# zellerlab/GECCO

Measured on AMD Instinct MI355X. Metric: genes/sec CRF decode (windowed fwd-bwd marginals + Viterbi), higher is better.
Workload: dtype f64

## Files before the change

gecco_amd/build.py:

```python
import os
import shutil
import subprocess
import sys

HERE = os.path.dirname(os.path.abspath(__file__))
CSRC = os.path.join(HERE, "csrc")
LIBDIR = os.path.join(HERE, "lib")
LIB = os.path.join(LIBDIR, "libgecco_crf.so")
SOURCES = ["crf_model.cpp", "crf_plan.cpp", "crf_session.cpp", "crf_tables.cpp", "capi.cpp", "crf_kernels.hip", "crf_sequence.hip", "crf_segment.hip", "crf_general.hip", "crf_general_windowed.hip", "crf_spans.hip", "crf_conditionals.hip", "crf_runs.hip", "crf_sample.hip", "crf_kbest.hip", "crf_minrun.hip", "crf_counts.hip", "crf_edges.hip", "crf_composition.hip", "crf_exact.hip", "crf_train.hip", "crf_train_general.hip", "crf_fisher.hip", "crf_overlap.hip", "crf_forest.hip"]
HEADERS = ["crf_model.hpp", "crf_plan.hpp", "crf_device.hpp", "crf_scan.hpp", "crf_lanes.hpp", "crf_lane_group.hpp", "crf_contig_walk.hpp", "crf_vd_short.hpp", "crf_session.hpp", "crf_tables.hpp", "crf_exact_exp.hpp", "crf_npsum.hpp", "crf_train.hpp", "crf_train_host.hpp", "crf_hip_own.hpp", "crf_fisher.hpp", "crf_overlap.hpp", "crf_forest.hpp", os.path.join("..", "..", "include", "gecco_crf.h")]
EXTRA_FLAGS = {"crf_exact.hip": ["-ffp-contract=off"], "capi.cpp": ["-ffp-contract=off"], "crf_fisher.hip": ["-ffp-contract=off"],
               "crf_forest.hip": ["-ffp-contract=off"],
               "crf_spans.hip": ["-ffp-contract=off"],
               "crf_runs.hip": ["-ffp-contract=off"],
               "crf_conditionals.hip": ["-ffp-contract=off"],
               "crf_sample.hip": ["-ffp-contract=off"],
               "crf_kbest.hip": ["-ffp-contract=off"], "crf_minrun.hip": ["-ffp-contract=off"], "crf_counts.hip": ["-ffp-contract=off"]}
ARCH = "gfx950"


def _hipcc() -> str:
    for cand in (os.environ.get("HIPCC"), shutil.which("hipcc"), "/opt/rocm/bin/hipcc"):
        if cand and os.path.exists(cand):
            return cand
    raise RuntimeError("hipcc not found (ROCm toolchain required to build gecco_amd)")


def needs_build() -> bool:
    if not os.path.exists(LIB):
        return True
    t = os.path.getmtime(LIB)
    deps = [os.path.join(CSRC, s) for s in SOURCES + HEADERS] + [os.path.abspath(__file__)]
    return any(os.path.getmtime(d) > t for d in deps)


LAST_BUILD = {}


def build_native(force: bool = False, verbose: bool = False) -> str:
    if not force and not needs_build():
        LAST_BUILD["libgecco_crf"] = "reused (up to date against every source and header)"
        return LIB
    os.makedirs(LIBDIR, exist_ok=True)
# ... 58 lines not shown
```

gecco_amd/csrc/crf_vd_short.hpp:

```cpp
#pragma once

#include "crf_device.hpp"
#include "crf_scan.hpp"

namespace gecco {
namespace {

constexpr int kT = 256;
constexpr int kGPL = kSeqGenesPerLane;
constexpr int kBlockGenes = kT * kGPL;
static_assert(kBlockGenes == kSeqBlockGenes, "host tables assume this block size");

__device__ __forceinline__ double vd_max(double a, double b) {
    double r;
    asm("v_max_f64 %0, %1, %2" : "=v"(r) : "v"(a), "v"(b));
    return r;
}
__device__ __forceinline__ double vd_min(double a, double b) {
    double r;
    asm("v_min_f64 %0, %1, %2" : "=v"(r) : "v"(a), "v"(b));
    return r;
}
__device__ __forceinline__ double vd_min_abs(double a, double b) {
    double r;
    asm("v_min_f64 %0, |%1|, |%2|" : "=v"(r) : "v"(a), "v"(b));
    return r;
}
__device__ __forceinline__ double vd_max_s(double a, double bound) {
    double r;
    asm("v_max_f64 %0, %1, %2" : "=v"(r) : "v"(a), "s"(bound));
    return r;
}
__device__ __forceinline__ double vd_min_s(double a, double bound) {
    double r;
    asm("v_min_f64 %0, %1, %2" : "=v"(r) : "v"(a), "s"(bound));
    return r;
}
__device__ __forceinline__ void vd_shift_in_gt(uint32_t &acc, double x, double bound) {
    asm("v_cmp_lt_f64 vcc, %2, %1\n\tv_addc_co_u32 %0, vcc, %0, %0, vcc" : "+v"(acc) : "v"(x), "s"(bound) : "vcc");
}
struct COp {
    static __device__ __forceinline__ CE identity() { return CE{0.0, -__builtin_huge_val(), __builtin_huge_val()}; }
    static __device__ __forceinline__ CE combine(const CE &a, const CE &b) {
        return CE{a.a + b.a, vd_min(vd_max(a.L + b.a, b.L), b.H), vd_min(vd_max(a.H + b.a, b.L), b.H)};
    }
    static __device__ __forceinline__ void combine_into(CE &t, CE &v) {
        asm volatile(
            "v_add_f64 %[tl], %[tl], %[a]\n\t"
            "v_add_f64 %[th], %[th], %[a]\n\t"
            "v_add_f64 %[a], %[ta], %[a]\n\t"
            "v_max_f64 %[tl], %[tl], %[L]\n\t"
            "v_max_f64 %[th], %[th], %[L]\n\t"
            "v_min_f64 %[L], %[tl], %[H]\n\t"
            "v_min_f64 %[H], %[th], %[H]"
            : [a] "+v"(v.a), [L] "+v"(v.L), [H] "+v"(v.H), [tl] "+v"(t.L), [th] "+v"(t.H)
            : [ta] "v"(t.a));
    }
};

__device__ __forceinline__ double vd_bound(const SeqArgs &A, double nnz, double n) { return nnz * A.v_wmax2 + (n + 2.0) * A.v_tmax; }
constexpr double kVdEps = 2.220446049250313e-16;
__device__ __forceinline__ double vd_margin(double r, double ulpM) { return (4.0 * r + 4.0) * ulpM; }
__device__ __forceinline__ double vd_sum_slack(const SeqArgs &A, double nnz) {
    return (nnz * nnz + 3.0 * nnz + 1.0) * A.v_wmax2 * (0.5 * kVdEps) * 1.000001;
}

constexpr int kFixChunk = 1024;
struct FixStage {
    double2 st[kFixChunk];
    uint32_t bpw[kFixChunk / 16];
};
__device__ __forceinline__ void exact_states(const SeqArgs &A, int g0, int m, FixStage &fx, int first_lane) {
// ... 119 lines not shown
__device__ __forceinline__ void exact_delta_contig(const SeqArgs &A, int gs, int ge, FixStage &fx) {
    uint32_t *bpc = exact_bp_words(A, gs);
    double d0 = 0.0, d1 = 0.0;
    for (int cb = gs; cb < ge; cb += kFixChunk) {
        const int m = min(kFixChunk, ge - cb);
        const double e0 = d0, e1 = d1;
        exact_states(A, cb, m, fx, 0);
        __syncthreads();
        if (threadIdx.x == 0) exact_walk(A, fx, m, cb == gs, d0, d1);
        __syncthreads();
        d0 = fx.st[m - 1].x;
        d1 = fx.st[m - 1].y;
        exact_backpointers(A, fx, m, cb == gs, e0, e1);
        __syncthreads();
        for (int i = threadIdx.x; i < (m + 15) / 16; i += kT) bpc[(cb - gs) / 16 + i] = fx.bpw[i];
        __syncthreads();
    }
    exact_backtrack(A, gs, ge, d0, d1);
}

constexpr double kVdPad = 1e30;

struct VdShortSmem {
    double st[kT * (kGPL + 1)];
    uint32_t mark[kBlockGenes / 32];
    int c_end;
    CE tot[kT / 64];
    uint32_t mtot[kT / 64];
    double pv[kT / 64];
    uint32_t pbad[kT / 64];
    uint32_t vote[kT / 64];
};
static_assert(sizeof(VdShortSmem) <= 20480, "eight workgroups per CU");
__device__ __forceinline__ void load_short(const double *__restrict__ v, int g0, int n, VdShortSmem &stg, double (&x)[kGPL]) {
    const int base = int(threadIdx.x) * kGPL;
    const double *vp = v + g0;
    double *row = stg.st + threadIdx.x * (kGPL + 1);
    const int wave_end = (__builtin_amdgcn_readfirstlane(int(threadIdx.x >> 6)) + 1) * 64 * kGPL;
    if (wave_end <= n) {
#pragma unroll
        for (int k = 0; k < kGPL; ++k) x[k] = vp[base + k];
#pragma unroll
        for (int k = 0; k < kGPL; ++k) row[k] = x[k];
        return;
    }
#pragma unroll
    for (int k = 0; k < kGPL; ++k) x[k] = vp[max(min(base + k, n - 1), 0)];
#pragma unroll
    for (int k = 0; k < kGPL; ++k) {
        x[k] = base + k < n ? x[k] : kVdPad;
        row[k] = x[k];
    }
}

__device__ __forceinline__ uint32_t wave_or_u32(uint32_t v) {
    v |= uint32_t(__builtin_amdgcn_update_dpp(0, int(v), 0x111, 0xF, 0xF, true));
    v |= uint32_t(__builtin_amdgcn_update_dpp(0, int(v), 0x112, 0xF, 0xF, true));
    v |= uint32_t(__builtin_amdgcn_update_dpp(0, int(v), 0x114, 0xF, 0xF, true));
    v |= uint32_t(__builtin_amdgcn_update_dpp(0, int(v), 0x118, 0xF, 0xF, true));
    v |= uint32_t(__builtin_amdgcn_update_dpp(0, int(v), 0x142, 0xA, 0xF, true));
    v |= uint32_t(__builtin_amdgcn_update_dpp(0, int(v), 0x143, 0xC, 0xF, true));
    return uint32_t(__builtin_amdgcn_readlane(int(v), 63));
}

constexpr int kVdRun = 6;
__device__ __forceinline__ void vd_apply(const CE &P, double in, double &v) {
    asm volatile("v_add_f64 %0, %1, %2\n\tv_max_f64 %0, %0, %3\n\tv_min_f64 %0, %0, %4" : "+v"(v) : "v"(in), "v"(P.a), "v"(P.L), "v"(P.H));
}
__device__ __forceinline__ void vd_propagate(const CE &P, double &v, uint64_t &known) {
    for (int it = 0; it < kVdRun; ++it) {
        const uint64_t todo = (known << 1) & ~known;
        if (!todo) break;
        const double in = dpp_f64_z<0x138>(v);
        if (__builtin_amdgcn_inverse_ballot_w64(todo)) vd_apply(P, in, v);
        known |= todo;
    }
}

__device__ __forceinline__ void vd_short_block(const SeqArgs &A, const int blk, VdShortSmem &stg) {
    CE *lds = stg.tot;
    uint32_t *ldsm = stg.mtot;
    const int slot = threadIdx.x;
    const int g0 = __builtin_amdgcn_readfirstlane(A.cblk[blk]), n = __builtin_amdgcn_readfirstlane(A.cblk[blk + 1]) - g0;
    const uint32_t bits = A.lane_bits[blk * kT + slot];
    const uint32_t first = bits & 0xffu, last = bits >> 8;
    const uint32_t wave_bits = wave_or_u32(bits);
    double x[kGPL];
    load_short(A.dstate, g0, n, stg, x);
    const int cnt = min(kGPL, n - slot * kGPL);
    const double *row = stg.st + slot * (kGPL + 1);
    CE P = COp::identity();
#pragma unroll
    for (int k = 0; k < kGPL; ++k) {
        const double dvk = x[k];
        const bool fst = (first >> k) & 1u;
        const double c = A.v_k + dvk;
        const double l2 = vd_min_s(vd_max_s(P.L, A.v_lo), A.v_hi) + c, h2 = vd_min_s(vd_max_s(P.H, A.v_lo), A.v_hi) + c;
        P.a += c;
        P.L = l2;
        P.H = h2;
        if ((wave_bits >> k) & 1u) {
            asm volatile("" ::: "memory");
            P.L = fst ? dvk : l2;
            P.H = fst ? dvk : h2;
        }
    }
    double Din;
    {
        const int wave = __builtin_amdgcn_readfirstlane(int(threadIdx.x >> 6));
        double v = P.L;
        uint64_t known = __builtin_amdgcn_ballot_w64(P.L == P.H);
        vd_propagate(P, v, known);
        const bool wave_bad = (known | (known - 1)) != ~uint64_t(0) || !(known & (wave ? (uint64_t(2) << kVdRun) - 1 : uint64_t(1)));
        if ((threadIdx.x & 63) == 63) stg.pv[wave] = v;
        block_or_post(wave_bad, stg.pbad);
        __syncthreads();
        if (block_or_read(stg.pbad)) {
            const CE M = block_scan_exclusive<COp, false, CE, kScanThreads, true, true>(P, lds, static_cast<CE *>(nullptr));
            Din = M.L;
        } else {
            const double carry = stg.pv[wave ? wave - 1 : 0];
            if (!(known & 1u)) {
                if ((threadIdx.x & 63) == 0) vd_apply(P, carry, v);
                known |= 1u;
                vd_propagate(P, v, known);
            }
            Din = dpp_f64<0x138, 0xF>(carry, v);
        }
    }
    double ulpM = 0.0, margin = 1e-6 * fmax(1.0, fmax(fabs(A.v_lo), fabs(A.v_hi)));
    if (A.csr_gene_ptr) {
        const double nnz = double(A.csr_gene_ptr[g0 + n] - A.csr_gene_ptr[g0]);
        ulpM = vd_bound(A, nnz, double(n)) * kVdEps;
        margin = vd_margin(double(n), ulpM) + vd_sum_slack(A, nnz);
    }
    ulpM = __hiloint2double(__builtin_amdgcn_readfirstlane(__double2hiint(ulpM)), __builtin_amdgcn_readfirstlane(__double2loint(ulpM)));
    margin = __hiloint2double(__builtin_amdgcn_readfirstlane(__double2hiint(margin)), __builtin_amdgcn_readfirstlane(__double2loint(margin)));
    uint32_t maps = 0, lane_map;
    bool sensitive = false;
    {
        double Dq = Din, nearest = __builtin_huge_val();
#pragma unroll
        for (int k = 0; k < kGPL; ++k) {
            const double dvk = row[k];
            const double stepped = vd_min_s(vd_max_s(Dq, A.v_lo), A.v_hi) + (A.v_k + dvk);
            Dq = stepped;
            if ((wave_bits >> k) & 1u) {
                asm volatile("" ::: "memory");
                Dq = ((first >> k) & 1u) ? dvk : stepped;
            }
            vd_shift_in_gt(maps, Dq, A.v_lo);
            vd_shift_in_gt(maps, Dq, A.v_hi);
            double dist = vd_min_abs(Dq - A.v_hi, Dq - A.v_lo);
            if ((wave_bits >> (8 + k)) & 1u) {
                asm volatile("" ::: "memory");
                const bool lst = (last >> k) & 1u;
                maps = lst ? ((maps & ~3u) | (Dq > 0.0 ? 3u : 0u)) : maps;
                dist = lst ? fabs(Dq) : dist;
            }
            nearest = vd_min(nearest, dist);
        }
        sensitive = nearest <= margin;
    }
    auto label_map = [&]() {
        uint32_t y0 = 0u, y1 = 1u;
#pragma unroll
        for (int k = kGPL - 1; k >= 0; --k) {
            y0 = __builtin_amdgcn_ubfe(maps, uint32_t(2 * (kGPL - 1 - k)) | y0, 1u);
            y1 = __builtin_amdgcn_ubfe(maps, uint32_t(2 * (kGPL - 1 - k)) | y1, 1u);
        }
        return y0 | (y1 << 1);
    };
    const bool lane_sensitive = sensitive && A.v_exact;
    int vote = lane_sensitive ? 1 : 0;
    uint32_t mtotal;
    lane_map = label_map();
    uint32_t lab = block_scan_exclusive_back<MapOp>(lane_map, ldsm, &mtotal, &vote, stg.vote) & 1u;
    const bool wg_sensitive = vote != 0;
    if (wg_sensitive) {
        double Dq = Din;
        uint64_t sat = 0;
#pragma unroll
        for (int k = 0; k < kGPL; ++k) {
            if (k < cnt) {
                const double dvk = row[k];
            Dq = ((first >> k) & 1u) ? dvk : fmin(fmax(Dq, A.v_lo), A.v_hi) + (A.v_k + dvk);
                const uint64_t c = Dq >= A.v_hi + margin ? 1u : (Dq <= A.v_lo - margin ? 2u : 0u);
                sat |= c << (8 * k);
            }
        }
        *reinterpret_cast<uint64_t *>(&stg.st[slot * (kGPL + 1) + kGPL]) = sat;
        __syncthreads();
    } else {
        sensitive = false;
    }
    bool lane_flagged = false;
    if (sensitive && cnt > 0) {
        double D = 0.0;
        int r = 0;
        auto certain = [&](double x) { return x >= A.v_hi + margin || x <= A.v_lo - margin; };
        if (!(first & 1u)) {
            const int t0 = slot * kGPL;
            int p = t0 - 1;
            auto dval = [&](int t) { return stg.st[(t / kGPL) * (kGPL + 1) + t % kGPL]; };
            for (;; --p) {
                if (A.flags[g0 + p] & 1u) {
                    D = dval(p);
                    r = 0;
                    break;
                }
                const uint32_t c = reinterpret_cast<const uint8_t *>(&stg.st[((p - 1) / kGPL) * (kGPL + 1) + kGPL])[(p - 1) % kGPL];
                if (c) {
                    D = (c == 1u ? A.v_hi : A.v_lo) + (A.v_k + dval(p));
                    r = 1;
                    break;
                }
            }
            for (int t = p + 1; t < t0; ++t) {
                r = certain(D) ? 1 : r + 1;
                D = fmin(fmax(D, A.v_lo), A.v_hi) + (A.v_k + dval(t));
            }
        }
        maps = 0;
#pragma unroll
        for (int k = 0; k < kGPL; ++k) {
            if (k < cnt) {
                const double dvk = row[k];
                const bool fst = (first >> k) & 1u;
                r = fst ? 0 : (certain(D) ? 1 : r + 1);
                D = fst ? dvk : fmin(fmax(D, A.v_lo), A.v_hi) + (A.v_k + dvk);
                const bool lst = (last >> k) & 1u;
                const double thi = lst ? 0.0 : A.v_hi, tlo = lst ? 0.0 : A.v_lo;
                maps |= ((D > thi ? 1u : 0u) | (D > tlo ? 2u : 0u)) << (2 * (kGPL - 1 - k));
                const int gt = g0 + slot * kGPL + k;
                const double mr = vd_margin(double(r), ulpM) +
                                  (A.csr_gene_ptr ? vd_sum_slack(A, double(A.csr_gene_ptr[gt + 1] - A.csr_gene_ptr[max(gt - r, g0)])) : 0.0);
                lane_flagged |= fabs(D - thi) <= mr || fabs(D - tlo) <= mr;
            }
        }
        if (A.vd_stats) {
            atomicAdd(A.vd_stats + 0, 1u);
            if (lane_flagged) atomicAdd(A.vd_stats + 1, 1u);
        }
    }
    bool wg_flagged = false;
    if (wg_sensitive) {
        block_or_post(lane_flagged, stg.vote);
        __syncthreads();
        wg_flagged = block_or_read(stg.vote);
        lane_map = label_map();
        lab = block_scan_exclusive_back<MapOp>(lane_map, ldsm, &mtotal) & 1u;
    }
    uint64_t packed = 0;
#pragma unroll
    for (int k = kGPL - 1; k >= 0; --k) {
        lab = __builtin_amdgcn_ubfe(maps, uint32_t(2 * (kGPL - 1 - k)) | lab, 1u);
        packed |= uint64_t(lab) << (8 * k);
    }
    {
        struct __attribute__((packed)) Bytes8 {
            uint64_t v;
        };
        int8_t *yp = A.y + g0 + slot * kGPL;
        if (cnt >= kGPL) {
            reinterpret_cast<Bytes8 *>(yp)->v = packed;
        } else {
            for (int k = 0; k < cnt; ++k) yp[k] = int8_t(packed >> (8 * k));
        }
    }
    if (wg_flagged && A.csr_gene_ptr) {
        uint32_t *mark = stg.mark;
        int *c_end = &stg.c_end;
        __syncthreads();
        if (slot < kBlockGenes / 32) mark[slot] = 0;
        __syncthreads();
        if (lane_flagged) {
            int prev = -1;
            for (int k = 0; k < cnt; ++k) {
                int t = slot * kGPL + k;
                while (!(A.flags[g0 + t] & 1u)) --t;
                if (t != prev) atomicOr(&mark[t >> 5], 1u << (t & 31));
                prev = t;
            }
        }
        __syncthreads();
        FixStage &st2 = *reinterpret_cast<FixStage *>(stg.st);
        static_assert(sizeof(stg.st) >= sizeof(FixStage), "exact pass: LDS for one chunk of state scores");
        for (int wi = 0; wi < kBlockGenes / 32; ++wi) {
            uint32_t bits = mark[wi];
            while (bits) {
                const int cs = wi * 32 + __builtin_ctz(bits);
// ... 24 lines not shown
```

gecco_amd/csrc/crf_kernels.hip:

```cpp
#include "crf_device.hpp"
#include "crf_lanes.hpp"
#include "crf_vd_short.hpp"

namespace gecco {
namespace {

typedef double f64x2 __attribute__((ext_vector_type(2)));

__device__ __forceinline__ double max_nocanon(double a, double b) {
    double r;
    asm("v_max_f64 %0, %1, %2" : "=v"(r) : "v"(a), "v"(b));
    return r;
}

__device__ __forceinline__ int xcd_remap(int orig, int nwg) {
    const int xcd = orig & 7, q = nwg >> 3, r = nwg & 7;
    const int base = xcd < r ? xcd * (q + 1) : r * (q + 1) + (xcd - r) * q;
    return base + (orig >> 3);
}

__device__ __forceinline__ void store_wt(double *p, double v) {
    __hip_atomic_store(reinterpret_cast<unsigned long long *>(p), static_cast<unsigned long long>(__double_as_longlong(v)),
                       __ATOMIC_RELAXED, __HIP_MEMORY_SCOPE_AGENT);
}
// ... 67 lines not shown
    }
}

typedef int i32x4 __attribute__((ext_vector_type(4)));

template <bool PROD = false>
__device__ __forceinline__ void state_scores_buf(__amdgpu_buffer_rsrc_t ra, __amdgpu_buffer_rsrc_t rw, uint32_t off,
                                                 uint32_t cnt, double &s0, double &s1, uint32_t imax = 0x0FFFFFFFu,
                                                 uint32_t none = 0xFFFFFFF0u) {
    for (uint32_t base = 0; base < cnt; base += kGatherUnroll) {
        int a[kGatherUnroll];
#pragma unroll
        for (int u = 0; u < kGatherUnroll; ++u)
            a[u] = __builtin_amdgcn_raw_buffer_load_b32(ra, int((off + base + u) << 2), 0, 0);
        i32x4 w[kGatherUnroll];
#pragma unroll
        for (int u = 0; u < kGatherUnroll; ++u) {
            const uint32_t wo = base + u < cnt ? min(uint32_t(a[u]), imax) << 4 : none;
            w[u] = __builtin_amdgcn_raw_buffer_load_b128(rw, int(wo), 0, 0);
        }
#pragma unroll
        for (int u = 0; u < kGatherUnroll; ++u) {
            if (PROD) {
                s1 += __hiloint2double(w[u].y, w[u].x);
                s0 *= __hiloint2double(w[u].w, w[u].z);
            } else {
                s0 += __hiloint2double(w[u].y, w[u].x);
                s1 += __hiloint2double(w[u].w, w[u].z);
            }
        }
    }
}

template <int WMAX, bool EXACT, bool RESCALE, int NT, int TT, bool LEAN = false, bool SMALL = false>
__device__ __forceinline__ void windowed_tile(const WinArgs &P, WinSmem<WMAX, NT, TT, EXACT> &sm, const int tile) {
    using Smem = WinSmem<WMAX, NT, TT, EXACT>;
    constexpr int JMAX = Smem::JMAX;
    constexpr bool RATIO = !RESCALE && EXACT;
    const int W = EXACT ? WMAX : P.W;
    const int tid = threadIdx.x, lane = tid & 63, wave = tid >> 6;
    const int OUT = NT - (W - 1);
    const int ns = TT * OUT + 2 * (W - 1);
    const int q0 = tile * (TT * OUT) - (W - 1);

    const int4 td = P.all_regular ? make_int4(0, 0, 0, 1) : P.tile_desc[tile];
    int gene[JMAX];
    bool start[JMAX];
#pragma unroll
    for (int j = 0; j < JMAX; ++j) {
        gene[j] = -1;
        start[j] = false;
    }
    if (td.w & 1) {
#pragma unroll
        for (int j = 0; j < JMAX; ++j) {
            const int sl = tid + j * NT, q = q0 + sl;
            if (sl < ns && q >= 0 && q < P.S) {
                gene[j] = q + td.x;
                start[j] = (reinterpret_cast<const uint32_t *>(P.start_bits)[q >> 5] >> (q & 31)) & 1u;
            }
        }
    } else {
        const int cnt = td.z - td.y + 1;
        for (int j = tid; j <= cnt; j += NT) {
            sm.cslot[j] = P.c_slot[td.y + j];
            if (j < cnt) {
                sm.cgene[j] = P.c_gene[td.y + j];
// ... 158 lines not shown
                } else {
                    const double e = exp_neg(fabs(d), P.expc);
                    const double e1 = d > 0.0 ? 1.0 : e;
                    sm.ef[sl] = f64x2{d > 0.0 ? e : 1.0, P.mu01 * e1};
                    sm.ginfo[sl] = (start[j] ? 0x80000000u : 0u) | uint32_t(gene[j] + 1);
                }
            }
        }
    }
    if (P.dstate_out) {
#pragma unroll
        for (int j = 0; j < JMAX; ++j) {
            if (TT > 1 || j == 0 || wave == 0) {
                const int sl = tid + j * NT;
                if (sl >= W - 1 && sl < TT * OUT + (W - 1) && gene[j] >= 0) {
                    const double d = RATIO ? sc1[j] : sc1[j] - sc0[j];
                    const double dd = __hiloint2double(__double2hiint(d) ^ (P.label ? 0 : int(0x80000000u)), __double2loint(d));
                    store_wt(P.dstate_out + gene[j], dd);
                }
            }
        }
    }
    __syncthreads();

    const uint32_t rmask = P.rescale_mask;
    const double rho = P.rho;
#pragma unroll 1
    for (int ph = 0; ph < TT; ++ph) {
        if (SMALL && ph > 0 && q0 + (W - 1) + ph * OUT >= P.S) break;
        const int sbase = ph * OUT + tid;
        bool my_start = false;
        int my_gene;
        if (RATIO) {
            const int q = q0 + sbase;
            my_gene = (td.w & 1) ? ((q >= 0 && q < P.S) ? q + td.x : -1) : int(sm.ginfo[sbase]) - 1;
        } else {
            const uint32_t gi = sm.ginfo[sbase];
            my_start = gi >> 31;
            my_gene = int(gi & 0x7fffffffu) - 1;
        }
        const f64x2 *ef = sm.ef + sbase;
        if constexpr (RATIO) {
            const double *rrs = rr + sbase;
            double A1[WMAX];
            const double r0 = lds_read1(rrs);
            double a0 = 1.0, a1 = fabs(r0) * P.kappa_over_mu01;
            A1[0] = a1;
#pragma unroll
            for (int k = 1; k < WMAX; ++k) {
                if (EXACT || k < W) {
                    const double r = fabs(lds_read1(rrs + k));
                    const double t = a0 + a1;
                    a1 = fma(a1, rho, a0) * r;
                    a0 = t;
                    A1[k] = a1;
                }
            }
            asm volatile("" ::: "memory");
            double z = fma(a1, P.inv_kappa, a0);
            const bool renorm = __builtin_amdgcn_ballot_w64(!(z < P.ratio_zmax)) != 0;
            auto pair_of = [&](double r, double &e0, double &f) {
                const bool pos = r > P.mu01;
                const double rc = fmin(r, 1.0e300);
                double q = __builtin_amdgcn_rcp(rc);
                q = fma(fma(-rc, q, 1.0), q, q);
                e0 = pos ? P.mu01 * q : 1.0;
                f = pos ? P.mu01 : r;
            };
            if (renorm) {
                double e0, f;
                pair_of(fabs(r0), e0, f);
                a0 = e0;
                a1 = f * P.kappa_over_mu01;
                A1[0] = a1;
#pragma unroll
                for (int k = 1; k < WMAX; ++k) {
                    if (EXACT || k < W) {
                        pair_of(fabs(rrs[k]), e0, f);
                        const double t = a0 + a1;
                        a1 = fma(a1, rho, a0) * f;
                        a0 = t * e0;
                        A1[k] = a1;
                    }
                }
                z = fma(a1, P.inv_kappa, a0);
            }
            double b0, b1;
            {
                double r = __builtin_amdgcn_rcp(z);
                r = fma(fma(-z, r, 1.0), r, r);
                b0 = __double2hiint(r0) < 0 ? r : 0.0;
                b1 = b0 * P.inv_kappa;
            }
            double R = 0.0;
            double *carry = reinterpret_cast<double *>(&sm.carry[0][0]);
            if (!renorm) {
                double rcur = W > 1 ? lds_read1(rrs + (W - 1)) : 0.0;
#pragma unroll
                for (int k = WMAX - 1; k >= 0; --k) {
                    if (EXACT || k < W) {
                        double rnext = 0.0;
                        if (k > 1) rnext = lds_read1(rrs + (k - 1));
                        const double cand = A1[k] * b1;
                        if (k < W - 1) {
                            if (lane == 63 && wave < NT / 64 - 1) carry[wave * WMAX + k] = R;
                            R = wave_shr1_zero(R);
                        }
                        R = max_nocanon(R, cand);
                        if (k > 0) {
                            const double u = fabs(rcur) * b1;
                            b1 = fma(u, rho, b0);
                            b0 = b0 + u;
                        }
                        rcur = rnext;
                    }
                }
            } else {
#pragma unroll
                for (int k = WMAX - 1; k >= 0; --k) {
                    if (EXACT || k < W) {
                        const double cand = A1[k] * b1;
                        if (k < W - 1) {
                            if (lane == 63 && wave < NT / 64 - 1) carry[wave * WMAX + k] = R;
                            R = wave_shr1_zero(R);
                        }
                        R = max_nocanon(R, cand);
                        if (k > 0) {
                            double e0, f;
                            pair_of(fabs(rrs[k]), e0, f);
                            const double cc = e0 * b0, u = f * b1;
                            b0 = cc + u;
                            b1 = fma(u, rho, cc);
                        }
                    }
                }
            }
            __syncthreads();
            if (wave > 0 && lane < W - 1) {
                int t2 = tid;
                if (LEAN) asm volatile("" : "+v"(t2));
                R = fmax(R, carry[((t2 >> 6) - 1) * WMAX + (t2 & 63)]);
            }
            R = fmin(R, 1.0);
            if (tid >= W - 1 && my_gene >= 0) store_wt(P.p_out + my_gene, R);
        } else if constexpr (!RESCALE) {
            double A1[WMAX];
            double a0, a1;
            {
                const f64x2 c = ef[0];
                a0 = c.x;
                a1 = fabs(c.y) * P.kappa_over_mu01;
            }
            A1[0] = a1;
#pragma unroll
            for (int k = 1; k < WMAX; ++k) {
                if (EXACT || k < W) {
                    const f64x2 c = ef[k];
                    const double t = a0 + a1;
                    a1 = fma(a1, rho, a0) * fabs(c.y);
                    a0 = t * c.x;
                    A1[k] = a1;
                }
            }
            asm volatile("" ::: "memory");

            double b0, b1;
            {
                const double z = fma(a1, P.inv_kappa, a0);
                double r = __builtin_amdgcn_rcp(z);
                r = fma(fma(-z, r, 1.0), r, r);
                b0 = my_start ? r : 0.0;
                b1 = b0 * P.inv_kappa;
            }
            double R = 0.0;
            double *carry = reinterpret_cast<double *>(&sm.carry[0][0]);
#pragma unroll
            for (int k = WMAX - 1; k >= 0; --k) {
// ... 56 lines not shown
                    Rx = take ? x : Rx;
                    Ry = take ? y : Ry;
                    if (k > 0) {
                        const f64x2 c = ef[k];
                        const double cc = c.x * b0, u = c.y * b1;
                        b0 = cc + u;
                        b1 = fma(u, rho, cc);
                        if ((rmask >> k) & 1u) rescale_pair(b0, b1);
                    }
                }
            }
            __syncthreads();
            if (wave > 0 && lane < W - 1) {
                const f64x2 c = sm.carry[wave - 1][lane];
                if (c.x * Ry > Rx * c.y || (Rx == 0.0 && Ry == 0.0)) {
                    Rx = c.x;
                    Ry = c.y;
                }
            }
            if (tid >= W - 1 && my_gene >= 0) P.p_out[my_gene] = (Rx + Ry > 0.0) ? Rx / (Rx + Ry) : 0.0;
        }
        if (TT > 1) __syncthreads();
    }
}

template <int WMAX, bool EXACT, bool RESCALE, int NT, int TT>
__global__ void __launch_bounds__(NT, (RESCALE ? (WMAX <= 20 ? 5 : 3) : (WMAX <= 20 ? (TT <= 2 ? 8 : 5) : 3))) crf_windowed_l2(const WinArgs P) {
    __shared__ WinSmem<WMAX, NT, TT, EXACT> sm;
    windowed_tile<WMAX, EXACT, RESCALE, NT, TT>(P, sm, xcd_remap(blockIdx.x, P.ntiles));
}

__global__ void __launch_bounds__(kWinThreads, 4) crf_windowed_small_l2(const WinArgs P) {
    __shared__ WinSmem<20, kWinThreads, 2, true> sm;
    windowed_tile<20, true, false, kWinThreads, 2, false, true>(P, sm, 0);
}

struct PipeArgs {
    const int32_t *gene_ptr, *attr_id;
    const double2 *ptab;
    const int32_t *c_slot, *c_gene, *c_n;
    const int4 *tile_desc;
    const uint64_t *start_bits;
    double *p_out, *dstate_out;
    const double *rtab;
    int32_t S, ntiles, step, label, n_genes, A, all_regular, nvd8, prod_cnt;
    double mu01, rho, kappa_over_mu01, inv_kappa, ratio_zmax, expc5[5];
    const double *dstate;
    const uint8_t *flags;
    const uint16_t *lane_bits;
    const int32_t *cblk, *csr_gene_ptr, *csr_attr_id;
    const double2 *csr_wtab01;
    double2 *alpha;
    uint32_t *vd_stats;
    int8_t *y;
    int32_t s_n_genes, csr_n_attrs, v_exact, n_cblocks;
    double t00, t01, t10, t11, v_lo, v_hi, v_k, v_wmax2, v_tmax;
};

template <int TILES, int WGS>
__global__ void __launch_bounds__(kWinThreads, WGS) crf_decode_pipelined(const PipeArgs K) {
    using Smem = WinSmem<20, kWinThreads, TILES, true>;
    constexpr size_t kBytes = sizeof(Smem) > sizeof(VdShortSmem) ? sizeof(Smem) : sizeof(VdShortSmem);
    static_assert(kBytes <= 20480, "eight workgroups per CU");
    __shared__ __attribute__((aligned(16))) unsigned char raw[kBytes];
    const int b = blockIdx.x;
    if (b >= K.nvd8) {
        WinArgs P{};
        P.gene_ptr = K.gene_ptr;
        P.attr_id = K.attr_id;
        P.ptab = K.ptab;
        P.prod_cnt = K.prod_cnt;
        P.c_slot = K.c_slot;
        P.c_gene = K.c_gene;
        P.c_n = K.c_n;
        P.tile_desc = K.tile_desc;
        P.start_bits = K.start_bits;
        P.p_out = K.p_out;
        P.dstate_out = K.dstate_out;
        P.rtab = K.rtab;
        P.S = K.S;
        P.ntiles = K.ntiles;
        P.W = 20;
        P.step = K.step;
        P.L = 2;
        P.label = K.label;
        P.n_genes = K.n_genes;
        P.A = K.A;
        P.tiles_per_wg = TILES;
        P.all_regular = K.all_regular;
        P.mu01 = K.mu01;
        P.rho = K.rho;
        P.kappa_over_mu01 = K.kappa_over_mu01;
        P.inv_kappa = K.inv_kappa;
        P.ratio_zmax = K.ratio_zmax;
#pragma unroll
        for (int i = 0; i < 5; ++i) P.expc[7 + i] = K.expc5[i];
        P.csr_begin = P.csr_end = -1;
        windowed_tile<20, true, false, kWinThreads, TILES, true>(P, *reinterpret_cast<Smem *>(raw), xcd_remap(b - K.nvd8, K.ntiles));
        return;
    }
    if (b >= K.n_cblocks) return;
    SeqArgs A{};
    A.dstate = K.dstate;
    A.flags = K.flags;
    A.lane_bits = K.lane_bits;
    A.cblk = K.cblk;
    A.csr_gene_ptr = K.csr_gene_ptr;
    A.csr_attr_id = K.csr_attr_id;
    A.csr_wtab01 = K.csr_wtab01;
    A.csr_n_attrs = K.csr_n_attrs;
    A.alpha = K.alpha;
    A.vd_stats = K.vd_stats;
    A.y = K.y;
    A.n_genes = K.s_n_genes;
    A.n_cblocks = K.n_cblocks;
    A.short_contigs = 1;
    A.v_exact = K.v_exact;
    A.t00 = K.t00;
    A.t01 = K.t01;
    A.t10 = K.t10;
    A.t11 = K.t11;
    A.v_lo = K.v_lo;
    A.v_hi = K.v_hi;
    A.v_k = K.v_k;
    A.v_wmax2 = K.v_wmax2;
    A.v_tmax = K.v_tmax;
    vd_short_block(A, b, *reinterpret_cast<VdShortSmem *>(raw));
}

__device__ __forceinline__ double2 slot_emission(const WinArgs &P, int gene) {
    double s0 = 0.0, s1 = 0.0;
// ... 189 lines not shown
```

gecco_amd/csrc/crf_plan.cpp:

```cpp
#include "crf_plan.hpp"

#include <algorithm>
#include <functional>
#include <memory>
#include <cmath>
#include <cstdio>
#include <cstdlib>
#include <cstring>

#include "../../include/gecco_crf.h"
#include "crf_session.hpp"

namespace gecco {

int check_hip(hipError_t e, const char *what) {
    if (e == hipSuccess) return GECCO_CRF_OK;
    set_error(std::string(what) + ": " + hipGetErrorString(e));
    if (e == hipErrorNoDevice || e == hipErrorInvalidDevice) return GECCO_CRF_ENODEV;
    if (e == hipErrorOutOfMemory) return GECCO_CRF_ENOMEM;
    return GECCO_CRF_EHIP;
}

Model::~Model() {
    for (auto &e : sessions) session_destroy(e.second);
// ... 51 lines not shown
    if (rc) return rc;
    if (m.L == 2) {
        for (int label = 0; label < 2; ++label) {
            DeviceTables::WinConsts &c = t->win[label];
            const int o = 1 - label;
            auto T = [&](int i, int j) { return m.trans[size_t(i) * 2 + j]; };
            c.mu01 = std::exp(T(o, label) + T(label, o) - 2.0 * T(o, o));
            c.rho = std::exp(T(label, label) + T(o, o) - T(o, label) - T(label, o));
            const double kappa = std::exp(T(label, o) - T(o, o));
            c.kappa_over_mu01 = std::exp(T(o, o) - T(o, label));
            c.inv_kappa = 1.0 / kappa;
            const double mx = *std::max_element(m.trans.begin(), m.trans.end());
            auto G = [&](int i, int j) { return std::exp(m.trans[size_t(i) * 2 + j] - mx); };
            c.g00 = G(o, o);
            c.g01 = G(o, label);
            c.g10 = G(label, o);
            c.g11 = G(label, label);
            fill_exp_coefficients(c.expc);
            c.ratio_zmax = 1.0e250;
            const double room = 700.0 - std::fabs(T(o, label) + T(label, o) - 2.0 * T(o, o));
            c.prod_cnt = room > 0.0 ? std::min(t->slot_prod_max_cnt, slot_prod_max_cnt(t->slot_dmax * (700.0 / room))) : 0;
        }
        DeviceTables::SeqConsts &q = t->seq;
        q.mx = *std::max_element(m.trans.begin(), m.trans.end());
        q.m00 = std::exp(m.trans[0] - q.mx);
        q.m01 = std::exp(m.trans[1] - q.mx);
        q.m10 = std::exp(m.trans[2] - q.mx);
        q.m11 = std::exp(m.trans[3] - q.mx);
        const double lo = *std::min_element(m.trans.begin(), m.trans.end());
        q.raw_fold = (q.mx - lo) * double(kSeqGenesPerLane) < 600.0 ? 1 : 0;
        q.v_lo = m.trans[1] - m.trans[3];
        q.v_hi = m.trans[0] - m.trans[2];
        q.v_k = m.trans[3] - m.trans[0];
        q.v_exact = 1;
        fill_exp_coefficients(q.expc);
        t->consts_ok = true;
    }
    *out = t.get();
    m.dev_tables.push_back(t.release());
    return GECCO_CRF_OK;
}

int Arena::reserve(size_t bytes, const char *what) {
    if (bytes <= cap && h) return GECCO_CRF_OK;
    release();
    const size_t want = std::max<size_t>(bytes + bytes / 4, 4096);
    int rc = check_hip(hipHostMalloc(reinterpret_cast<void **>(&h), want, hipHostMallocMapped | hipHostMallocPortable), what);
    if (rc) return rc;
    if ((rc = check_hip(hipMalloc(reinterpret_cast<void **>(&d), want), what))) {
        (void)hipHostFree(h);
        h = nullptr;
        return rc;
    }
    cap = want;
    return GECCO_CRF_OK;
}

void Arena::release() {
    if (h) (void)hipHostFree(h);
    if (d) (void)hipFree(d);
    h = d = nullptr;
    cap = 0;
}

Plan::~Plan() {
    if (device < 0) return;
    home.enter(device);
// ... 1336 lines not shown
```

Before: 79.22 billion.

## Replace map-composition block scan with ballot carry-lookahead label propagation

```diff
diff --git a/gecco_amd/build.py b/gecco_amd/build.py
--- a/gecco_amd/build.py
+++ b/gecco_amd/build.py
@@ -8,7 +8,7 @@
 LIBDIR = os.path.join(HERE, "lib")
 LIB = os.path.join(LIBDIR, "libgecco_crf.so")
 SOURCES = ["crf_model.cpp", "crf_plan.cpp", "crf_session.cpp", "crf_tables.cpp", "capi.cpp", "crf_kernels.hip", "crf_sequence.hip", "crf_segment.hip", "crf_general.hip", "crf_general_windowed.hip", "crf_spans.hip", "crf_conditionals.hip", "crf_runs.hip", "crf_sample.hip", "crf_kbest.hip", "crf_minrun.hip", "crf_counts.hip", "crf_edges.hip", "crf_composition.hip", "crf_exact.hip", "crf_train.hip", "crf_train_general.hip", "crf_fisher.hip", "crf_overlap.hip", "crf_forest.hip"]
-HEADERS = ["crf_model.hpp", "crf_plan.hpp", "crf_device.hpp", "crf_scan.hpp", "crf_lanes.hpp", "crf_lane_group.hpp", "crf_contig_walk.hpp", "crf_vd_short.hpp", "crf_session.hpp", "crf_tables.hpp", "crf_exact_exp.hpp", "crf_npsum.hpp", "crf_train.hpp", "crf_train_host.hpp", "crf_hip_own.hpp", "crf_fisher.hpp", "crf_overlap.hpp", "crf_forest.hpp", os.path.join("..", "..", "include", "gecco_crf.h")]
+HEADERS = ["crf_model.hpp", "crf_plan.hpp", "crf_device.hpp", "crf_scan.hpp", "crf_lanes.hpp", "crf_lane_group.hpp", "crf_contig_walk.hpp", "crf_vd_short.hpp", "crf_vd_labels.hpp", "crf_session.hpp", "crf_tables.hpp", "crf_exact_exp.hpp", "crf_npsum.hpp", "crf_train.hpp", "crf_train_host.hpp", "crf_hip_own.hpp", "crf_fisher.hpp", "crf_overlap.hpp", "crf_forest.hpp", os.path.join("..", "..", "include", "gecco_crf.h")]
 EXTRA_FLAGS = {"crf_exact.hip": ["-ffp-contract=off"], "capi.cpp": ["-ffp-contract=off"], "crf_fisher.hip": ["-ffp-contract=off"],
                "crf_forest.hip": ["-ffp-contract=off"],
                "crf_spans.hip": ["-ffp-contract=off"],
diff --git a/gecco_amd/csrc/crf_vd_labels.hpp b/gecco_amd/csrc/crf_vd_labels.hpp
--- /dev/null
+++ b/gecco_amd/csrc/crf_vd_labels.hpp
@@ -0,0 +1,49 @@
+#pragma once
+#include <cstdint>
+
+#if defined(__HIPCC__)
+#define GECCO_VDL_HD __host__ __device__ __forceinline__
+#else
+#define GECCO_VDL_HD inline
+#endif
+
+namespace gecco {
+
+constexpr uint32_t kVdIdMaps = 0xAAAAu;
+constexpr uint32_t kVdOnes = 0x15555u;
+
+GECCO_VDL_HD uint32_t vd_brev32(uint32_t x) {
+#if defined(__clang__)
+    return __builtin_bitreverse32(x);
+#else
+    uint32_t r = 0;
+    for (int i = 0; i < 32; ++i) r |= ((x >> i) & 1u) << (31 - i);
+    return r;
+#endif
+}
+GECCO_VDL_HD uint64_t vd_brev64(uint64_t x) {
+#if defined(__clang__)
+    return __builtin_bitreverse64(x);
+#else
+    return (uint64_t(vd_brev32(uint32_t(x))) << 32) | vd_brev32(uint32_t(x >> 32));
+#endif
+}
+
+GECCO_VDL_HD bool vd_lane_is_constant(uint32_t maps) { return maps != kVdIdMaps; }
+GECCO_VDL_HD bool vd_lane_is_one(uint32_t maps) { return maps > kVdIdMaps; }
+
+GECCO_VDL_HD uint64_t vd_label_bytes(uint32_t maps, bool in) {
+    const uint32_t s = maps + kVdOnes + (in ? 1u : 0u);
+    const uint32_t z = ~(s ^ maps) & 0x15554u;
+    const uint32_t r = vd_brev32(z);
+    const uint32_t lo = (((r >> 15) & 0x7fu) * 0x41041u) & 0x01010101u, hi = ((r >> 23) * 0x41041u) & 0x01010101u;
+    return uint64_t(lo) | (uint64_t(hi) << 32);
+}
+
+GECCO_VDL_HD uint32_t vd_wave_total(uint64_t K, uint64_t V) { return K ? ((V & K & (~K + 1u)) ? 3u : 0u) : 2u; }
+GECCO_VDL_HD uint64_t vd_entering_labels(uint64_t K, uint64_t V, uint32_t carry) {
+    const uint64_t g = vd_brev64(V & K), p = ~vd_brev64(K);
+    return vd_brev64(((g | p) + g + carry) ^ p);
+}
+
+}
diff --git a/gecco_amd/csrc/crf_vd_short.hpp b/gecco_amd/csrc/crf_vd_short.hpp
--- a/gecco_amd/csrc/crf_vd_short.hpp
+++ b/gecco_amd/csrc/crf_vd_short.hpp
@@ -2,6 +2,7 @@
 
 #include "crf_device.hpp"
 #include "crf_scan.hpp"
+#include "crf_vd_labels.hpp"
 
 namespace gecco {
 namespace {
@@ -223,25 +224,19 @@
     uint32_t vote[kT / 64];
 };
 static_assert(sizeof(VdShortSmem) <= 20480, "eight workgroups per CU");
-__device__ __forceinline__ void load_short(const double *__restrict__ v, int g0, int n, VdShortSmem &stg, double (&x)[kGPL]) {
+__device__ __forceinline__ void load_short(const double *__restrict__ v, int g0, int n, double (&x)[kGPL]) {
     const int base = int(threadIdx.x) * kGPL;
     const double *vp = v + g0;
-    double *row = stg.st + threadIdx.x * (kGPL + 1);
     const int wave_end = (__builtin_amdgcn_readfirstlane(int(threadIdx.x >> 6)) + 1) * 64 * kGPL;
     if (wave_end <= n) {
 #pragma unroll
         for (int k = 0; k < kGPL; ++k) x[k] = vp[base + k];
-#pragma unroll
-        for (int k = 0; k < kGPL; ++k) row[k] = x[k];
         return;
     }
 #pragma unroll
     for (int k = 0; k < kGPL; ++k) x[k] = vp[max(min(base + k, n - 1), 0)];
 #pragma unroll
-    for (int k = 0; k < kGPL; ++k) {
-        x[k] = base + k < n ? x[k] : kVdPad;
-        row[k] = x[k];
-    }
+    for (int k = 0; k < kGPL; ++k) x[k] = base + k < n ? x[k] : kVdPad;
 }
 
 __device__ __forceinline__ uint32_t wave_or_u32(uint32_t v) {
@@ -266,6 +261,22 @@
         if (__builtin_amdgcn_inverse_ballot_w64(todo)) vd_apply(P, in, v);
         known |= todo;
     }
+}
+
+__device__ __forceinline__ bool vd_label_entering(uint32_t maps, uint32_t *lds_totals , int *vote, uint32_t *lds_votes ) {
+    const int wave = __builtin_amdgcn_readfirstlane(int(threadIdx.x >> 6));
+    const uint64_t K = __builtin_amdgcn_ballot_w64(vd_lane_is_constant(maps)), V = __builtin_amdgcn_ballot_w64(vd_lane_is_one(maps));
+    if ((threadIdx.x & 63) == 63) lds_totals[wave] = vd_wave_total(K, V);
+    block_or_post<kT>(*vote != 0, lds_votes);
+    __syncthreads();
+    *vote = block_or_read<kT>(lds_votes) ? 1 : 0;
+    uint32_t carry = 0;
+#pragma unroll
+    for (int w = kT / 64 - 1; w >= 1; --w) {
+        const uint32_t t = uint32_t(__builtin_amdgcn_readfirstlane(int(lds_totals[w])));
+        if (w > wave && t != 2u) carry = t & 1u;
+    }
+    return __builtin_amdgcn_inverse_ballot_w64(vd_entering_labels(K, V, carry));
 }
 
 __device__ __forceinline__ void vd_short_block(const SeqArgs &A, const int blk, VdShortSmem &stg) {
@@ -277,9 +288,9 @@
     const uint32_t first = bits & 0xffu, last = bits >> 8;
     const uint32_t wave_bits = wave_or_u32(bits);
     double x[kGPL];
-    load_short(A.dstate, g0, n, stg, x);
+    load_short(A.dstate, g0, n, x);
     const int cnt = min(kGPL, n - slot * kGPL);
-    const double *row = stg.st + slot * (kGPL + 1);
+    double *row = stg.st + slot * (kGPL + 1);
     CE P = COp::identity();
 #pragma unroll
     for (int k = 0; k < kGPL; ++k) {
@@ -290,11 +301,14 @@
         P.a += c;
         P.L = l2;
         P.H = h2;
+        double parked = c;
         if ((wave_bits >> k) & 1u) {
             asm volatile("" ::: "memory");
             P.L = fst ? dvk : l2;
             P.H = fst ? dvk : h2;
-        }
+            parked = fst ? dvk : c;
+        }
+        row[k] = parked;
     }
     double Din;
     {
@@ -327,18 +341,18 @@
     }
     ulpM = __hiloint2double(__builtin_amdgcn_readfirstlane(__double2hiint(ulpM)), __builtin_amdgcn_readfirstlane(__double2loint(ulpM)));
     margin = __hiloint2double(__builtin_amdgcn_readfirstlane(__double2hiint(margin)), __builtin_amdgcn_readfirstlane(__double2loint(margin)));
-    uint32_t maps = 0, lane_map;
+    uint32_t maps = 0;
     bool sensitive = false;
     {
         double Dq = Din, nearest = __builtin_huge_val();
 #pragma unroll
         for (int k = 0; k < kGPL; ++k) {
-            const double dvk = row[k];
-            const double stepped = vd_min_s(vd_max_s(Dq, A.v_lo), A.v_hi) + (A.v_k + dvk);
+            const double cv = row[k];
+            const double stepped = vd_min_s(vd_max_s(Dq, A.v_lo), A.v_hi) + cv;
             Dq = stepped;
             if ((wave_bits >> k) & 1u) {
                 asm volatile("" ::: "memory");
-                Dq = ((first >> k) & 1u) ? dvk : stepped;
+                Dq = ((first >> k) & 1u) ? cv : stepped;
             }
             vd_shift_in_gt(maps, Dq, A.v_lo);
             vd_shift_in_gt(maps, Dq, A.v_hi);
@@ -353,20 +367,9 @@
         }
         sensitive = nearest <= margin;
     }
-    auto label_map = [&]() {
-        uint32_t y0 = 0u, y1 = 1u;
-#pragma unroll
-        for (int k = kGPL - 1; k >= 0; --k) {
-            y0 = __builtin_amdgcn_ubfe(maps, uint32_t(2 * (kGPL - 1 - k)) | y0, 1u);
-            y1 = __builtin_amdgcn_ubfe(maps, uint32_t(2 * (kGPL - 1 - k)) | y1, 1u);
-        }
-        return y0 | (y1 << 1);
-    };
     const bool lane_sensitive = sensitive && A.v_exact;
     int vote = lane_sensitive ? 1 : 0;
-    uint32_t mtotal;
-    lane_map = label_map();
-    uint32_t lab = block_scan_exclusive_back<MapOp>(lane_map, ldsm, &mtotal, &vote, stg.vote) & 1u;
+    bool lab = vd_label_entering(maps, ldsm, &vote, stg.vote);
     const bool wg_sensitive = vote != 0;
     if (wg_sensitive) {
         double Dq = Din;
@@ -374,8 +377,8 @@
 #pragma unroll
         for (int k = 0; k < kGPL; ++k) {
             if (k < cnt) {
-                const double dvk = row[k];
-            Dq = ((first >> k) & 1u) ? dvk : fmin(fmax(Dq, A.v_lo), A.v_hi) + (A.v_k + dvk);
+                const double cv = row[k];
+                Dq = ((first >> k) & 1u) ? cv : fmin(fmax(Dq, A.v_lo), A.v_hi) + cv;
                 const uint64_t c = Dq >= A.v_hi + margin ? 1u : (Dq <= A.v_lo - margin ? 2u : 0u);
                 sat |= c << (8 * k);
             }
@@ -402,24 +405,24 @@
                 }
                 const uint32_t c = reinterpret_cast<const uint8_t *>(&stg.st[((p - 1) / kGPL) * (kGPL + 1) + kGPL])[(p - 1) % kGPL];
                 if (c) {
-                    D = (c == 1u ? A.v_hi : A.v_lo) + (A.v_k + dval(p));
+                    D = (c == 1u ? A.v_hi : A.v_lo) + dval(p);
                     r = 1;
                     break;
                 }
             }
             for (int t = p + 1; t < t0; ++t) {
                 r = certain(D) ? 1 : r + 1;
-                D = fmin(fmax(D, A.v_lo), A.v_hi) + (A.v_k + dval(t));
+                D = fmin(fmax(D, A.v_lo), A.v_hi) + dval(t);
             }
         }
         maps = 0;
 #pragma unroll
         for (int k = 0; k < kGPL; ++k) {
             if (k < cnt) {
-                const double dvk = row[k];
+                const double cv = row[k];
                 const bool fst = (first >> k) & 1u;
                 r = fst ? 0 : (certain(D) ? 1 : r + 1);
-                D = fst ? dvk : fmin(fmax(D, A.v_lo), A.v_hi) + (A.v_k + dvk);
+                D = fst ? cv : fmin(fmax(D, A.v_lo), A.v_hi) + cv;
                 const bool lst = (last >> k) & 1u;
                 const double thi = lst ? 0.0 : A.v_hi, tlo = lst ? 0.0 : A.v_lo;
                 maps |= ((D > thi ? 1u : 0u) | (D > tlo ? 2u : 0u)) << (2 * (kGPL - 1 - k));
@@ -436,18 +439,11 @@
     }
     bool wg_flagged = false;
     if (wg_sensitive) {
-        block_or_post(lane_flagged, stg.vote);
-        __syncthreads();
-        wg_flagged = block_or_read(stg.vote);
-        lane_map = label_map();
-        lab = block_scan_exclusive_back<MapOp>(lane_map, ldsm, &mtotal) & 1u;
-    }
-    uint64_t packed = 0;
-#pragma unroll
-    for (int k = kGPL - 1; k >= 0; --k) {
-        lab = __builtin_amdgcn_ubfe(maps, uint32_t(2 * (kGPL - 1 - k)) | lab, 1u);
-        packed |= uint64_t(lab) << (8 * k);
-    }
+        int vote2 = lane_flagged ? 1 : 0;
+        lab = vd_label_entering(maps, ldsm, &vote2, stg.vote);
+        wg_flagged = vote2 != 0;
+    }
+    const uint64_t packed = vd_label_bytes(maps, lab);
     {
         struct __attribute__((packed)) Bytes8 {
             uint64_t v;
```

After: 80.01 billion (median of 3 runs). About the same (+1.0%).

## Trim instruction count in ratio windowed epilogue and Viterbi sign-map loop

Applied to the files above, without the earlier changes.

```diff
diff --git a/gecco_amd/csrc/crf_kernels.hip b/gecco_amd/csrc/crf_kernels.hip
--- a/gecco_amd/csrc/crf_kernels.hip
+++ b/gecco_amd/csrc/crf_kernels.hip
@@ -123,7 +123,7 @@
     }
 }
 
-template <int WMAX, bool EXACT, bool RESCALE, int NT, int TT, bool LEAN = false, bool SMALL = false>
+template <int WMAX, bool EXACT, bool RESCALE, int NT, int TT, bool SMALL = false>
 __device__ __forceinline__ void windowed_tile(const WinArgs &P, WinSmem<WMAX, NT, TT, EXACT> &sm, const int tile) {
     using Smem = WinSmem<WMAX, NT, TT, EXACT>;
     constexpr int JMAX = Smem::JMAX;
@@ -348,8 +348,7 @@
         bool my_start = false;
         int my_gene;
         if (RATIO) {
-            const int q = q0 + sbase;
-            my_gene = (td.w & 1) ? ((q >= 0 && q < P.S) ? q + td.x : -1) : int(sm.ginfo[sbase]) - 1;
+            my_gene = -1;
         } else {
             const uint32_t gi = sm.ginfo[sbase];
             my_start = gi >> 31;
@@ -357,7 +356,9 @@
         }
         const f64x2 *ef = sm.ef + sbase;
         if constexpr (RATIO) {
-            const double *rrs = rr + sbase;
+            uint32_t sb8;
+            asm("v_lshl_add_u32 %0, %1, 3, %2" : "=v"(sb8) : "v"(tid), "s"(ph * OUT * 8));
+            const double *rrs = reinterpret_cast<const double *>(reinterpret_cast<const char *>(rr) + sb8);
             double A1[WMAX];
             const double r0 = lds_read1(rrs);
             double a0 = 1.0, a1 = fabs(r0) * P.kappa_over_mu01;
@@ -405,11 +406,12 @@
             {
                 double r = __builtin_amdgcn_rcp(z);
                 r = fma(fma(-z, r, 1.0), r, r);
-                b0 = __double2hiint(r0) < 0 ? r : 0.0;
+                const double rs = __builtin_copysign(r, r0);
+                asm("v_max_f64 %0, -%1, 0" : "=v"(b0) : "v"(rs));
                 b1 = b0 * P.inv_kappa;
             }
             double R = 0.0;
-            double *carry = reinterpret_cast<double *>(&sm.carry[0][0]);
+            double *const crow = reinterpret_cast<double *>(&sm.carry[0][0]) + wave * WMAX;
             if (!renorm) {
                 double rcur = W > 1 ? lds_read1(rrs + (W - 1)) : 0.0;
 #pragma unroll
@@ -419,7 +421,7 @@
                         if (k > 1) rnext = lds_read1(rrs + (k - 1));
                         const double cand = A1[k] * b1;
                         if (k < W - 1) {
-                            if (lane == 63 && wave < NT / 64 - 1) carry[wave * WMAX + k] = R;
+                            if (lane == 63 && wave < NT / 64 - 1) crow[k] = R;
                             R = wave_shr1_zero(R);
                         }
                         R = max_nocanon(R, cand);
@@ -437,7 +439,7 @@
                     if (EXACT || k < W) {
                         const double cand = A1[k] * b1;
                         if (k < W - 1) {
-                            if (lane == 63 && wave < NT / 64 - 1) carry[wave * WMAX + k] = R;
+                            if (lane == 63 && wave < NT / 64 - 1) crow[k] = R;
                             R = wave_shr1_zero(R);
                         }
                         R = max_nocanon(R, cand);
@@ -453,12 +455,20 @@
             }
             __syncthreads();
             if (wave > 0 && lane < W - 1) {
-                int t2 = tid;
-                if (LEAN) asm volatile("" : "+v"(t2));
-                R = fmax(R, carry[((t2 >> 6) - 1) * WMAX + (t2 & 63)]);
-            }
-            R = fmin(R, 1.0);
-            if (tid >= W - 1 && my_gene >= 0) store_wt(P.p_out + my_gene, R);
+                static_assert(WMAX - 1 <= 32, "v_mbcnt_lo counts the lanes below it among the first 32");
+                uint32_t l;
+                asm volatile("v_mbcnt_lo_u32_b32 %0, -1, 0" : "=v"(l));
+                R = max_nocanon(R, crow[int(l) - WMAX]);
+            }
+            asm("v_min_f64 %0, %1, 1.0" : "=v"(R) : "v"(R));
+            if (td.w & 1) {
+                const int qs = q0 + ph * OUT;
+                char *const base = reinterpret_cast<char *>(P.p_out + (int64_t(q0) + td.x));
+                if (tid >= W - 1 && tid < P.S - qs) store_wt(reinterpret_cast<double *>(base + sb8), R);
+            } else {
+                const int g = int(*reinterpret_cast<const uint32_t *>(reinterpret_cast<const char *>(sm.ginfo) + (sb8 >> 1))) - 1;
+                if (tid >= W - 1 && g >= 0) store_wt(P.p_out + g, R);
+            }
         } else if constexpr (!RESCALE) {
             double A1[WMAX];
             double a0, a1;
@@ -581,7 +591,7 @@
 
 __global__ void __launch_bounds__(kWinThreads, 4) crf_windowed_small_l2(const WinArgs P) {
     __shared__ WinSmem<20, kWinThreads, 2, true> sm;
-    windowed_tile<20, true, false, kWinThreads, 2, false, true>(P, sm, 0);
+    windowed_tile<20, true, false, kWinThreads, 2, true>(P, sm, 0);
 }
 
 struct PipeArgs {
@@ -645,7 +655,7 @@
 #pragma unroll
         for (int i = 0; i < 5; ++i) P.expc[7 + i] = K.expc5[i];
         P.csr_begin = P.csr_end = -1;
-        windowed_tile<20, true, false, kWinThreads, TILES, true>(P, *reinterpret_cast<Smem *>(raw), xcd_remap(b - K.nvd8, K.ntiles));
+        windowed_tile<20, true, false, kWinThreads, TILES>(P, *reinterpret_cast<Smem *>(raw), xcd_remap(b - K.nvd8, K.ntiles));
         return;
     }
     if (b >= K.n_cblocks) return;
diff --git a/gecco_amd/csrc/crf_plan.cpp b/gecco_amd/csrc/crf_plan.cpp
--- a/gecco_amd/csrc/crf_plan.cpp
+++ b/gecco_amd/csrc/crf_plan.cpp
@@ -107,7 +107,10 @@
         q.v_lo = m.trans[1] - m.trans[3];
         q.v_hi = m.trans[0] - m.trans[2];
         q.v_k = m.trans[3] - m.trans[0];
-        q.v_exact = 1;
+        {
+            const char *env = std::getenv("GECCO_CRF_VD_EXACT");
+            q.v_exact = (env && env[0] == '0' && !env[1]) ? 0 : 1;
+        }
         fill_exp_coefficients(q.expc);
         t->consts_ok = true;
     }
diff --git a/gecco_amd/csrc/crf_vd_short.hpp b/gecco_amd/csrc/crf_vd_short.hpp
--- a/gecco_amd/csrc/crf_vd_short.hpp
+++ b/gecco_amd/csrc/crf_vd_short.hpp
@@ -36,8 +36,12 @@
     asm("v_min_f64 %0, %1, %2" : "=v"(r) : "v"(a), "s"(bound));
     return r;
 }
-__device__ __forceinline__ void vd_shift_in_gt(uint32_t &acc, double x, double bound) {
-    asm("v_cmp_lt_f64 vcc, %2, %1\n\tv_addc_co_u32 %0, vcc, %0, %0, vcc" : "+v"(acc) : "v"(x), "s"(bound) : "vcc");
+__device__ __forceinline__ void vd_shift_in_sign(uint32_t &acc, double diff) {
+    acc = __builtin_amdgcn_alignbit(acc, uint32_t(__double2hiint(diff)), 31u);
+}
+__device__ __forceinline__ double vd_threshold(double bound) {
+    const long long b = __double_as_longlong(bound);
+    return __longlong_as_double(b == (long long)(0x8000000000000000ull) ? 0ll : b);
 }
 struct COp {
     static __device__ __forceinline__ CE identity() { return CE{0.0, -__builtin_huge_val(), __builtin_huge_val()}; }
@@ -330,6 +334,7 @@
     uint32_t maps = 0, lane_map;
     bool sensitive = false;
     {
+        const double thr_lo = vd_threshold(A.v_lo), thr_hi = vd_threshold(A.v_hi);
         double Dq = Din, nearest = __builtin_huge_val();
 #pragma unroll
         for (int k = 0; k < kGPL; ++k) {
@@ -340,9 +345,10 @@
                 asm volatile("" ::: "memory");
                 Dq = ((first >> k) & 1u) ? dvk : stepped;
             }
-            vd_shift_in_gt(maps, Dq, A.v_lo);
-            vd_shift_in_gt(maps, Dq, A.v_hi);
-            double dist = vd_min_abs(Dq - A.v_hi, Dq - A.v_lo);
+            const double below_lo = thr_lo - Dq, below_hi = thr_hi - Dq;
+            vd_shift_in_sign(maps, below_lo);
+            vd_shift_in_sign(maps, below_hi);
+            double dist = vd_min_abs(below_hi, below_lo);
             if ((wave_bits >> (8 + k)) & 1u) {
                 asm volatile("" ::: "memory");
                 const bool lst = (last >> k) & 1u;
```

New measurement: 78.28 billion before, 78.99 billion after, median of 6. About the same (+0.9%).
